# Lumina-Group/libzkp

Hardware: AMD Instinct MI355X
Metric: proofs/sec (whole node) + ms/proof p50, 4096-proof mixed batch (range / equality / membership / improvement) per MI355X (higher is better)
Workload: dtype u32/u64 integer limbs (10x25.5-bit GF(2^255-19), BN254 Fq on 9x29-bit limbs in the MSM loops and 10x26-bit elsewhere, 8x32-bit Fr and scalars mod l, 2x64-bit f128)

## Files before the change

__graft_entry__.py:

```python
import ctypes
import os
import re
import subprocess
import sys

ROOT = os.path.dirname(os.path.abspath(__file__))
CSRC = os.path.join(ROOT, "libzkp_amd", "csrc")
LIB = os.path.join(ROOT, "libzkp_amd", "lib", "libzkp_hip.so")
ORACLE_LIB = os.path.join(ROOT, "oracle", "_build", "libzkp_oracle.so")
EMUL_DIR = os.path.join(ROOT, "tests", "emul")


def _newer(target, sources):
    if not os.path.exists(target):
        return False
    t = os.path.getmtime(target)
    return all(os.path.getmtime(s) <= t for s in sources)


def _run(cmd, **kw):
    print("+", " ".join(cmd), flush=True)
    subprocess.check_call(cmd, **kw)


# ... 51 lines not shown
        _run(["g++", "-O2", "-std=c++17", "-fPIC", "-shared", "-o", so, src])


def build_emul_qap_lanes(force=False):
    out = os.path.join(EMUL_DIR, "_build")
    os.makedirs(out, exist_ok=True)
    exe, src = os.path.join(out, "emul_g16_qap_lanes"), os.path.join(EMUL_DIR, "emul_g16_qap_lanes.cpp")
    hdrs = [os.path.join(CSRC, f) for f in os.listdir(CSRC) if f.endswith(".h")]
    if force or not _newer(exe, hdrs + [src]):
        _run(["g++", "-O1", "-g", "-std=c++17", "-fsanitize=address,undefined", "-fno-sanitize-recover=undefined", "-o", exe, src])
    return exe


def build_emul_composites_seal_program(force=False):
    out = os.path.join(EMUL_DIR, "_build")
    os.makedirs(out, exist_ok=True)
    exe, src = os.path.join(out, "emul_composites_seal"), os.path.join(EMUL_DIR, "emul_composites_seal.cpp")
    hdrs = [os.path.join(CSRC, f) for f in os.listdir(CSRC) if f.endswith(".h")]
    if force or not _newer(exe, hdrs + [src]):
        _run(["g++", "-O1", "-g", "-std=c++17", "-fsanitize=address,undefined", "-fno-sanitize-recover=undefined", "-o", exe, src])
    return exe


def build_devtier(force=False):
    d = os.path.join(ROOT, "tests", "devtier")
    out = os.path.join(d, "_build")
    os.makedirs(out, exist_ok=True)
    hipcc = os.environ.get("HIPCC", "/opt/rocm/bin/hipcc")
    so = os.path.join(out, "libdevtier.so")
    if not os.path.exists(LIB):
        build_hip()
    if force or unit_is_stale(so, so + ".d", base=ROOT) or not _newer(so, [LIB]):
        _run([hipcc, "-O3", "-std=c++17", "--offload-arch=gfx950", "-fPIC", "-shared", "-MMD", "-MF", so + ".d", os.path.relpath(os.path.join(d, "devtier.hip"), ROOT), "-o", so,
              "-L" + os.path.dirname(LIB), "-lzkp_hip", "-Wl,-rpath,$ORIGIN/../../../libzkp_amd/lib"], cwd=ROOT)
    return so


def build_abi_caller(force=False):
    src = os.path.join(ROOT, "tests", "abi", "abi_call_all.cpp")
    out = os.path.join(ROOT, "tests", "abi", "_build")
    exe = os.path.join(out, "abi_call_all")
    os.makedirs(out, exist_ok=True)
    if force or not _newer(exe, [src, os.path.join(ROOT, "include", "libzkp_hip.h"), LIB]):
        _run(["g++", "-O1", "-std=c++17", "-pthread", "-D__HIP_PLATFORM_AMD__", "-I/opt/rocm/include", src, "-o", exe, "-L" + os.path.dirname(LIB), "-lzkp_hip",
              "-L/opt/rocm/lib", "-lamdhip64", "-Wl,-rpath,$ORIGIN/../../../libzkp_amd/lib", "-Wl,-rpath,/opt/rocm/lib"])
    return exe
# ... 21 lines not shown
        _run(["g++", "-O1", "-std=c++17", "-pthread", "-D__HIP_PLATFORM_AMD__", "-I/opt/rocm/include", src, "-o", exe, "-L" + os.path.dirname(LIB), "-lzkp_hip",
              "-L/opt/rocm/lib", "-lamdhip64", "-Wl,-rpath,$ORIGIN/../../../libzkp_amd/lib", "-Wl,-rpath,/opt/rocm/lib"])
    return exe


def build_abi_seal_caller(force=False):
    src = os.path.join(ROOT, "tests", "abi", "abi_call_seal.cpp")
    out = os.path.join(ROOT, "tests", "abi", "_build")
    exe = os.path.join(out, "abi_call_seal")
    os.makedirs(out, exist_ok=True)
    hdrs = [os.path.join(ROOT, "include", h) for h in ("libzkp_hip.h", "libzkp_hip_seal.h", "libzkp_hip_composites.h")]
    if force or not _newer(exe, [src, LIB] + hdrs):
        _run(["g++", "-O1", "-std=c++17", "-pthread", src, "-o", exe, "-L" + os.path.dirname(LIB), "-lzkp_hip",
              "-L/opt/rocm/lib", "-lamdhip64", "-Wl,-rpath,$ORIGIN/../../../libzkp_amd/lib", "-Wl,-rpath,/opt/rocm/lib"])
    return exe


def build():
    build_hip()
    build_oracle()
    build_emul()
    build_emul_qap_lanes()
    build_emul_composites_seal_program()
    build_devtier()
    build_abi_caller()
    build_abi_verify_caller()
    build_abi_statements_caller()
    build_abi_seal_caller()
    sys.path.insert(0, ROOT)
    import libzkp_amd
    from libzkp_amd import _native
    L = ctypes.CDLL(_native.LIB_PATH)
    for sym in _native.EXPORTS + _native.EXPORTS_VERIFY + _native.EXPORTS_BP_LOCALISE + _native.EXPORTS_COMPOSITES + _native.EXPORTS_STATEMENTS + _native.EXPORTS_SEAL:
        getattr(L, sym)
    print("build ok:", _native.LIB_PATH)


def smoke():
    import numpy as np
    sys.path.insert(0, ROOT)
    from libzkp_amd import _native
    L = _native.lib()
    _native.check(L.zkp_hip_init(0), "zkp_hip_init")
    orc = ctypes.CDLL(ORACLE_LIB)
    orc.zkp_oracle_init()
    n = 8
# ... 53 lines not shown
```

libzkp_amd/csrc/batch_impl.inc:

```
namespace {

struct PackView {
    uint32_t n;
    const uint64_t* src_off;
    const uint32_t* len_fixed;
    const uint32_t* dyn_ix;
    const uint8_t* dyn_kind;
    const int32_t* status_fixed;
    const uint32_t* dyn_len; const int32_t* dyn_status;
    uint32_t* len; int32_t* status; uint64_t* out_off;
    const uint8_t* arena; uint8_t* out;
};
__global__ void __launch_bounds__(256) k_batch_lens(PackView P) {
    const uint32_t i = blockIdx.x * 256 + threadIdx.x;
    if (i >= P.n) return;
    int32_t st = P.status_fixed[i];
    uint32_t l = P.len_fixed[i];
    if (st == 0 && l == LEN_DYN) {
        const uint32_t k = P.dyn_ix[i];
        l = P.dyn_len[k];
        if (P.dyn_kind[i] == DYN_LEN_STATUS) st = P.dyn_status[k];
        else if (l == 0) st = ZKP_HIP_PROOF_GENERATION_FAILED;
    }
    if (st != 0) l = 0;
// ... 199 lines not shown
    V.n = P.n; V.src_off = (const uint64_t*)(in + P.i_src); V.len_fixed = (const uint32_t*)(in + P.i_lenf); V.dyn_ix = (const uint32_t*)(in + P.i_dix);
    V.dyn_kind = in + P.i_dkind; V.status_fixed = (const int32_t*)(in + P.i_stf); V.dyn_len = (const uint32_t*)(ar + P.a_dlen); V.dyn_status = (const int32_t*)(ar + P.a_dst);
    V.len = (uint32_t*)(P.d_meta + P.m_len); V.status = (int32_t*)(P.d_meta + P.m_status); V.out_off = (uint64_t*)(P.d_meta + P.m_off);
    V.arena = ar; V.out = P.d_out;
    return V;
}

int launch_shard_enqueue(ShardPlan& P) {
    BatchState* BS = nullptr; int rc;
    if ((rc = batch_state(&BS))) return rc;
    const uint32_t n = P.n;
    uint32_t lane_ix = 0;
    if ((rc = pick_lane(*BS, &lane_ix))) return rc;
    BatchLane& LN = BS->lane[lane_ix];
    hipStream_t st = LN.main;
    uint8_t *in = P.d_in, *ar = P.d_arena;
    const VariantPlan &R = P.var[ZKP_HIP_OP_RANGE], &E = P.var[ZKP_HIP_OP_EQUALITY], &T = P.var[ZKP_HIP_OP_THRESHOLD], &M = P.var[ZKP_HIP_OP_MEMBERSHIP],
                      &I = P.var[ZKP_HIP_OP_IMPROVEMENT], &C = P.var[ZKP_HIP_OP_CONSISTENCY];
    trace_origin(st);
    if (P.arena_bytes) HIP_TRY(hipMemsetAsync(ar, 0, P.arena_bytes, st));
    if (T.rows) HIP_TRY(hipMemcpyAsync(ar + T.arena, P.thr_img.data(), P.thr_img.size(), hipMemcpyHostToDevice, st));
    if (C.rows) HIP_TRY(hipMemcpyAsync(ar + C.arena, P.con_img.data(), P.con_img.size(), hipMemcpyHostToDevice, st));
    HIP_TRY(hipEventRecord(LN.go, st));
    bool used[4] = {false, false, false, false};
    auto on_stream = [&](int k, auto body) -> int {
        hipStream_t s = nullptr; used[k] = true;
        int rcs;
        if ((rcs = lane_stream(*BS, k, &s))) return rcs;
        HIP_TRY(hipStreamWaitEvent(s, LN.go, 0));
        if ((rcs = body(s))) return rcs;
        HIP_TRY(hipEventRecord(LN.done[k], s));
        return 0;
    };
    if (R.rows || T.rows || C.rows) {
        static const int edg_prio = env_int("ZKP_HIP_EDG_PRIORITY", 1);
        struct PrioScope { int& r; PrioScope(int& ref, int v) : r(ref) { r = v; } ~PrioScope() { r = 0; } };
        PrioScope prio(dev().msm_prio_now, (E.rows + M.rows) && edg_prio ? 1 : 0);
        SubBatch& jobs_sb = dev().sub[0];
        if ((rc = on_stream(0, [&](hipStream_t s) -> int {
                int rcb;
                if (R.rows && (rcb = prove_range_device_locked(R.rows, (const uint64_t*)(in + P.i_rv), (const uint64_t*)(in + P.i_rmin), (const uint64_t*)(in + P.i_rmax), 6, in + P.i_rseed,
                                                               ar + R.arena, R.stride, (uint32_t*)(ar + P.a_dlen), (int32_t*)(ar + P.a_dst), s, nullptr, (int)lane_ix))) return rcb;
                if (T.rows && (rcb = run_jobs_on(jobs_sb, P.thrJ, in + P.i_tseed, ar + T.arena, 6, s))) return rcb;
                if (C.rows) {
                    if ((rcb = run_jobs_on(jobs_sb, P.conJ, in + P.i_cseed, ar + C.arena, 6, s))) return rcb;
                    k_consistency_digest<<<(C.rows + 63) / 64, 64, 0, s>>>(ar + C.arena, C.stride, (const uint32_t*)(in + P.i_ccount), (const uint32_t*)(in + P.i_clen), C.rows);
// ... 332 lines not shown
```

libzkp_amd/csrc/edg_kernels.hip:

```cpp
#include "edg_launch.h"
#include "msm_kernel.h"

struct EdGather {
    static constexpr uint32_t ACC_W = GE_W, DIG_PER_WORD = 2;
    static __device__ __forceinline__ int32_t digit(uint32_t word, uint32_t w) { return (int32_t)(int16_t)(word >> (16 * (w & 1u))); }
    using Acc = ge;
    static __device__ __forceinline__ Acc identity() { return ge_identity(); }
    static constexpr uint32_t GATHER_WAVES = 3; static constexpr int GATHER_PREFETCH = 2;
    static constexpr uint32_t GATHER_W = EDG_ENTRY_W, GATHER_STRIDE = EDG_SLOT_W, GATHER_PRIO = 0;
    using GAcc = ge;
    static __device__ __forceinline__ GAcc to_gather(const ge& a) { return a; }
    static __device__ __forceinline__ ge from_gather(const GAcc& a) { return a; }
    static __device__ __forceinline__ GAcc accumulate_entry(const GAcc& acc, int32_t d, const uint32_t* e) { return edg_accumulate(acc, d, e); }
    static __device__ __forceinline__ void store(uint32_t* p, uint32_t idx, uint32_t row, uint32_t rows, const Acc& a) { st_ge(p, idx, row, rows, a); }
    static __device__ __forceinline__ Acc load(const uint32_t* p, uint32_t idx, uint32_t row, uint32_t rows) { return ld_ge(p, idx, row, rows); }
    static __device__ __forceinline__ Acc add(const Acc& a, const Acc& b) { return ge_add(a, b); }
};
template __global__ void k_msm_gather<EdGather>(MsmView, uint32_t, uint32_t);
struct EdGatherPrio : EdGather { static constexpr uint32_t GATHER_PRIO = 1; };
template __global__ void k_msm_gather<EdGatherPrio>(MsmView, uint32_t, uint32_t);

uint32_t edg_msm_rows_per_block() { return 256; }
uint32_t edg_msm_blocks_per_cu() {
    int occ = 0;
    if (hipOccupancyMaxActiveBlocksPerMultiprocessor(&occ, k_msm_gather<EdGather>, 256, gather_lds_bytes<EdGather>()) != hipSuccess) { (void)hipGetLastError(); return 0; }
    return occ > 0 ? (uint32_t)occ : 0;
}
void edg_launch_msm(const MsmView& m, uint32_t ngroups, uint32_t nblocks, hipStream_t st, bool raised) {
    const uint32_t grid = ((nblocks + 7) / 8) * 8;
    if (raised) k_msm_gather<EdGatherPrio><<<grid, 256, gather_lds_bytes<EdGather>(), st>>>(m, ngroups, nblocks);
    else k_msm_gather<EdGather><<<grid, 256, gather_lds_bytes<EdGather>(), st>>>(m, ngroups, nblocks);
}

template <uint32_t WB> __global__ void __launch_bounds__(64) k_edg_bases(const uint32_t* gens, uint32_t* bases) {
    const uint32_t b = blockIdx.x * 64 + threadIdx.x;
    if (b < NBASE) edg_step_bases(edg_geom(WB), gens, bases, b);
}
template <uint32_t WB> __global__ void __launch_bounds__(64) k_edg_starts(const uint32_t* bases, uint32_t* starts) {
    constexpr EdgGeom g = edg_geom(WB);
    const uint32_t bw = blockIdx.x * 64 + threadIdx.x;
    if (bw < NBASE * g.nwin) edg_step_starts(g, bases, starts, bw);
}
template <uint32_t WB> __global__ void __launch_bounds__(256) k_edg_fill(const uint32_t* bases, const uint32_t* starts, uint32_t* table) {
    constexpr EdgGeom g = edg_geom(WB);
    const uint32_t t = blockIdx.x * 256 + threadIdx.x;
    if (t < NBASE * g.nwin * g.nseg) edg_step_fill(g, bases, starts, table, t / g.nseg, t % g.nseg);
}
template <uint32_t WB> __global__ void __launch_bounds__(256) k_edg_affine(uint32_t* table) {
    constexpr EdgGeom g = edg_geom(WB);
    const size_t grp = (size_t)blockIdx.x * 256 + threadIdx.x;
    if (grp < (size_t)NBASE * g.nwin * g.nent / EDG_INV) edg_step_affine(table, grp);
}
template <uint32_t WB> __global__ void __launch_bounds__(256) k_edg_check(const uint32_t* table, const uint32_t* gens, int* bad) {
    constexpr EdgGeom g = edg_geom(WB);
// ... 29 lines not shown
```

libzkp_amd/csrc/edg_launch.h:

```cpp
#pragma once
#include <hip/hip_runtime.h>
#include "edg.h"

uint32_t edg_msm_rows_per_block();
uint32_t edg_msm_blocks_per_cu();
void edg_launch_msm(const zkp::MsmView& m, uint32_t ngroups, uint32_t nblocks, hipStream_t st, bool raised = false);
void edg_launch_build(const zkp::EdgGeom& g, const uint32_t* d_gens, uint32_t* d_table, uint32_t* d_scratch, int* d_bad, hipStream_t st);
size_t edg_build_scratch_words(const zkp::EdgGeom& g);
void edg_launch_sum(const zkp::ReduceView& R, uint32_t* sums, hipStream_t st);
```

libzkp_amd/csrc/g16_impl.inc:

```

namespace {

struct G16Key {
    bool loaded = false;
    uint32_t n_inst = 0, n_wit = 0, nv = 0, n_rows = 0, m = 0, logm = 0;
    G16Circuit C{};
    std::vector<void*> allocs;
    uint32_t *table_g1 = nullptr, *table_g2 = nullptr;
    G16Radix rx = g16_radix(G16_WBITS_DEFAULT);
    int shared_tables = -1;
    uint64_t table_bytes = 0;
    struct Chunking { DevLayout lay; const uint32_t* corr = nullptr; const uint16_t* scal = nullptr; };
    std::vector<SlotList> targets_g1, targets_g2;
    std::vector<uint16_t> hscal_g1, hscal_g2;
    std::map<uint64_t, Chunking> lays_g1, lays_g2;
    uint64_t win_g1 = 0, win_g2 = 0;
    const uint32_t *init_g1 = nullptr, *init_g2 = nullptr;
    G16Vk vk{}; bool vk_ready = false;
    uint64_t vk_table_bytes = 0;
    bool verifier_only() const { return vk_ready && !loaded; }
    const uint32_t *vm_kconst = nullptr, *vm_lines = nullptr;
};
struct G16Run {
    void* buf = nullptr; size_t cap = 0; hipStream_t side = nullptr, side2 = nullptr; hipEvent_t ev[4] = {nullptr, nullptr, nullptr, nullptr};
// ... 355 lines not shown
    auto put = [](std::vector<uint8_t>& v, const uint8_t* p, size_t n) { v.insert(v.end(), p, p + n); };
    auto put_len = [](std::vector<uint8_t>& v, uint64_t n) { for (int i = 0; i < 8; i++) v.push_back((uint8_t)(n >> (8 * i))); };
    size_t o_abc = 3, o_a = o_abc + T.n_inst, o_b = o_a + nv, o_h = o_b + nv, o_l = o_h + (m - 1);
    vk.clear();
    put(vk, g1at(0), 64); put(vk, g2at(0), 128); put(vk, g2at(1), 128); put(vk, g2at(2), 128);
    put_len(vk, T.n_inst); put(vk, g1at(o_abc), 64ull * T.n_inst);
    pk = vk;
    put(pk, g1at(1), 64); put(pk, g1at(2), 64);
    put_len(pk, nv); put(pk, g1at(o_a), 64ull * nv);
    put_len(pk, nv); put(pk, g1at(o_b), 64ull * nv);
    put_len(pk, nv); put(pk, g2at(3), 128ull * nv);
    put_len(pk, m - 1); put(pk, g1at(o_h), 64ull * (m - 1));
    put_len(pk, T.n_wit); put(pk, g1at(o_l), 64ull * T.n_wit);
    return load_key_locked(kind, pk.data(), pk.size());
}

int launch_msm_key(bool g2, const G16Radix& rx, const G16Key::Chunking& ch, const uint32_t* table, const uint32_t* acc_init, uint32_t rows, const uint32_t* digits, uint32_t* partial, hipStream_t st) {
    const DevLayout& D = ch.lay;
    const MsmView m = g16_msm_view(rx, D, ch.scal, table, acc_init, rows, digits, partial);
    Device::KProf& K = dev().prof[g2 ? 2 : 1];
    hipEvent_t e1 = nullptr;
    int rc = prof_begin(K, st, &e1);
    if (rc) return rc;
    ZKP_TRACED(g2 ? "k_msm_gather<G2Msm>" : "k_msm_gather<G1Msm>", st, g16_launch_msm(g2, m, st));
    prof_end(K, st, e1, D.adds_per_row * rows);
    return 0;
}


int run_g16(int kind, uint32_t rows, const uint64_t* d_value, const uint64_t* d_set_vals, const uint32_t* d_set_len, const uint8_t* d_seeds,
            uint8_t* d_out, uint64_t stride, hipStream_t st, uint32_t lane = 0) {
    G16Key& K = g16s().key[kind];
    if (!K.loaded) return no_proving_key(K);
    const uint32_t nsc = g16_nscalars(K.nv, K.m);
    const G16Key::Chunking *c1 = nullptr, *c1c = nullptr, *c2 = nullptr;
    int rc;
    if ((rc = get_chunking(K, false, G16_PART_AB, rows, &c1)) || (rc = get_chunking(K, true, G16_PART_ALL, rows, &c2))) return rc;
    if ((rc = get_chunking(K, false, G16_PART_C, rows, &c1c))) return rc;
    size_t off = 0;
    auto sz = [&](size_t bytes) { size_t o = off; off += align_up(bytes); return o; };
    const size_t W = (size_t)32 * rows;
    const size_t o_z = sz(W * K.nv), o_sd = sz((size_t)K.rx.digw * 4 * rows * nsc), o_rs = sz(W * 2), o_p1 = sz((size_t)c1->lay.nchunks * G1_JAC_W * 4 * rows),
                 o_p1c = sz((size_t)c1c->lay.nchunks * G1_JAC_W * 4 * rows), o_p2 = sz((size_t)c2->lay.nchunks * G2_JAC_W * 4 * rows),
                 o_s1 = sz((size_t)3 * G1_JAC_W * 4 * rows), o_s2 = sz((size_t)G2_JAC_W * 4 * rows), o_t1 = sz((size_t)G16_CPARTS * G1_JAC_W * 4 * rows),
                 o_qe = sz((size_t)3 * 36 * K.m * rows);
    G16Run& RW = g16s().run[kind][lane & 1u];
    if (off > RW.cap) {
// ... 365 lines not shown
```

libzkp_amd/csrc/g16_kernels.hip:

```cpp
#include "g16_launch.h"
#include "msm_kernel.h"

struct G1Msm {
    static constexpr uint32_t ACC_W = G1_JAC_W, DIG_PER_WORD = 2;
    static __device__ __forceinline__ int32_t digit(uint32_t word, uint32_t w) { return (int32_t)(int16_t)(word >> (16 * (w & 1u))); }
    using Acc = g1_jac;
    static __device__ __forceinline__ Acc identity() { return jac_infinity<fq>(); }
    static constexpr uint32_t GATHER_WAVES = 3; static constexpr int GATHER_PREFETCH = 2;
    static constexpr uint32_t GATHER_W = 16, GATHER_STRIDE = 16, GATHER_PRIO = 0;
    using GAcc = g1_xyzz9;
    static __device__ __forceinline__ GAcc to_gather(const g1_jac& a) { return xyzz9_from_jac(a); }
    static __device__ __forceinline__ g1_jac from_gather(const GAcc& a) { return jac_from_xyzz9(a); }
    static __device__ __forceinline__ GAcc accumulate_entry(const GAcc& acc, int32_t d, const uint32_t* e) {
        g1_aff9 q{fq9_unpack8(e), fq9_unpack8(e + 8)};
        q.y = fq9_select(d < 0, fq9_neg_k<4>(q.y), q.y);
        return g1_mmadd9(acc, q);
    }
    static __device__ __forceinline__ void store(uint32_t* p, uint32_t idx, uint32_t row, uint32_t rows, const Acc& a) { st_g1_jac(p, idx, row, rows, a); }
    static __device__ __forceinline__ Acc load(const uint32_t* p, uint32_t idx, uint32_t row, uint32_t rows) { return ld_g1_jac(p, idx, row, rows); }
    static __device__ __forceinline__ Acc add(const Acc& a, const Acc& b) { return jac_add(a, b); }
};
struct G2Msm {
    static constexpr uint32_t ACC_W = G2_JAC_W, DIG_PER_WORD = 2;
    static __device__ __forceinline__ int32_t digit(uint32_t word, uint32_t w) { return (int32_t)(int16_t)(word >> (16 * (w & 1u))); }
// ... 133 lines not shown
#define QAP_PASS(D, N, H, T) if (dif == D && nst == N && head == H && tail == T) { k_g16_qap_pass<D, N, H, T><<<grid, QAP_TB, 0, st>>>(V, C, h, poly0); return; }
        G16_QAP_LANE_VARIANTS(QAP_PASS)
#undef QAP_PASS
        ok = false;
    });
    return ok ? hipSuccess : hipErrorInvalidValue;
}
void g16_launch_cparts(const G16View& V, const uint32_t* sum_g1, uint32_t* tmp_g1, hipStream_t st) {
    k_g16_cparts<<<dim3((V.rows + TW - 1) / TW, G16_CPARTS), TW, 0, st>>>(V, sum_g1, tmp_g1);
}
void g16_launch_final(const G16View& V, const uint32_t* sum_g1, const uint32_t* sum_g2, const uint32_t* tmp_g1, hipStream_t st) {
    k_g16_final<<<dim3((V.rows + TW - 1) / TW, 3), TW, 0, st>>>(V, sum_g1, sum_g2, tmp_g1);
}
void g16_launch_mimc(const uint64_t* values, uint32_t n, const uint32_t* mimc_c, uint8_t* out, hipStream_t st) { k_mimc_commit<<<(n + TW - 1) / TW, TW, 0, st>>>(values, n, mimc_c, out); }
void g16_launch_build_table(bool g2, const uint32_t* bases, uint32_t nslots, uint32_t* table, hipStream_t st, bool msm_form, const G16Radix& rx) {
    const uint32_t seg_len = rx.nent < G16_TABLE_SEG ? rx.nent : G16_TABLE_SEG;
    const uint32_t threads = nslots * (rx.slot_ent / seg_len);
    if (!g2) k_g16_build_table<fq, 20><<<(threads + TW - 1) / TW, TW, 0, st>>>(bases, nslots, table, msm_form ? 1u : 0u, rx);
    else k_g16_build_table<fq2, 40><<<(threads + TW - 1) / TW, TW, 0, st>>>(bases, nslots, table, msm_form ? 1u : 0u, rx);
}
uint32_t g16_table_entry_words(bool g2, bool msm_form) { return msm_form ? (g2 ? G2Msm::GATHER_W : G1Msm::GATHER_W) : (g2 ? 40u : 20u); }
uint32_t g16_msm_rows_per_block(bool) { return 256u; }
uint32_t g16_msm_blocks_per_cu(bool g2) { return g2 ? G2Msm::GATHER_WAVES : G1Msm::GATHER_WAVES; }
void g16_launch_msm(bool g2, const MsmView& m, hipStream_t st) {
    const uint32_t ngroups = (m.rows + 255u) / 256u, nblocks = m.nchunks * ngroups, grid = ((nblocks + 7) / 8) * 8;
    if constexpr (gather_lds_bytes<G2Msm>() > 0 || gather_lds_bytes<G1Msm>() > 0) {
        if (gather_lds_bytes<G1Msm>()) (void)hipFuncSetAttribute(reinterpret_cast<const void*>(k_msm_gather<G1Msm>), hipFuncAttributeMaxDynamicSharedMemorySize, (int)gather_lds_bytes<G1Msm>());
        if (gather_lds_bytes<G2Msm>()) (void)hipFuncSetAttribute(reinterpret_cast<const void*>(k_msm_gather<G2Msm>), hipFuncAttributeMaxDynamicSharedMemorySize, (int)gather_lds_bytes<G2Msm>());
    }
    if (!g2) k_msm_gather<G1Msm><<<grid, 256, gather_lds_bytes<G1Msm>(), st>>>(m, ngroups, nblocks);
    else k_msm_gather<G2Msm><<<grid, 256, gather_lds_bytes<G2Msm>(), st>>>(m, ngroups, nblocks);
}
void g16_launch_sum(bool g2, const ReduceView& R, uint32_t* sums, hipStream_t st) {
    const dim3 grid((R.rows + G16_SUM_ROWS - 1) / G16_SUM_ROWS, R.ntargets);
    if (!g2) k_sum_t<G1Msm, G16_SUM_ROWS, G16_SUM_TB><<<grid, G16_SUM_TB, 0, st>>>(R, sums);
    else k_sum_t<G2Msm, G16_SUM_ROWS, G16_SUM_TB><<<grid, G16_SUM_TB, 0, st>>>(R, sums);
}
void g16_launch_serialize(bool g2, const uint32_t* jac, uint32_t rows, uint8_t* out, hipStream_t st) { k_g16_serialize<<<(rows + TW - 1) / TW, TW, 0, st>>>(g2, jac, rows, out); }
```

libzkp_amd/csrc/g16_launch.h:

```cpp
#pragma once
#include <hip/hip_runtime.h>
#include "g16_steps.h"
#include "bp_steps.h"

void g16_launch_witness(const zkp::G16View& V, hipStream_t st);
void g16_launch_zdigits(const zkp::G16View& V, hipStream_t st);
hipError_t g16_launch_qap(const zkp::G16View& V, const zkp::G16Circuit& C, hipStream_t st);
void g16_launch_cparts(const zkp::G16View& V, const uint32_t* sum_g1, uint32_t* tmp_g1, hipStream_t st);
void g16_launch_final(const zkp::G16View& V, const uint32_t* sum_g1, const uint32_t* sum_g2, const uint32_t* tmp_g1, hipStream_t st);
void g16_launch_mimc(const uint64_t* values, uint32_t n, const uint32_t* mimc_c, uint8_t* out, hipStream_t st);
void g16_launch_build_table(bool g2, const uint32_t* bases, uint32_t nslots, uint32_t* table, hipStream_t st, bool msm_form, const zkp::G16Radix& rx);
uint32_t g16_table_entry_words(bool g2, bool msm_form);
uint32_t g16_msm_rows_per_block(bool g2);
uint32_t g16_msm_blocks_per_cu(bool g2);
void g16_launch_msm(bool g2, const zkp::MsmView& m, hipStream_t st);
void g16_launch_sum(bool g2, const zkp::ReduceView& R, uint32_t* sums, hipStream_t st);
void g16_launch_serialize(bool g2, const uint32_t* jac, uint32_t rows, uint8_t* out, hipStream_t st);
```

libzkp_amd/csrc/msm_kernel.h:

```cpp
#pragma once
#include <hip/hip_runtime.h>
#include "bp_steps.h"

using namespace zkp;
static constexpr int TW = 64;
static constexpr int TB = 256;


template <class T> constexpr size_t gather_lds_bytes() { return T::GATHER_PREFETCH < 0 ? (size_t)4 * 2 * (T::GATHER_W / 4) * 64 * 16 : 0; }
template <class T>
__global__ void __launch_bounds__(256, T::GATHER_WAVES) k_msm_gather(MsmView m, uint32_t ngroups, uint32_t nblocks) {
    constexpr uint32_t V4 = T::GATHER_W / 4;
    constexpr uint32_t SV4 = T::GATHER_STRIDE / 4;
    const uint32_t tid = threadIdx.x;
    const uint32_t per_xcd = (nblocks + 7) / 8;
    const uint32_t linear = (blockIdx.x & 7u) * per_xcd + (blockIdx.x >> 3);
    if (linear >= nblocks) return;
    const uint32_t chunk = linear / ngroups, group = linear % ngroups;
    const uint32_t row = group * 256u + tid;
    const bool active = row < m.rows;
    const uint32_t st0 = m.chunk_step0[chunk], left = m.chunk_step0[chunk + 1] - st0;
    const uint2* const steps = reinterpret_cast<const uint2*>(m.steps) + st0;
    typename T::GAcc acc = T::to_gather(m.acc_init ? T::load(m.acc_init, 0, 0, 1) : T::identity());
    const uint4* const table4 = reinterpret_cast<const uint4*>(m.table);
    auto digit_word = [&](const uint2 ds) -> uint32_t { return active ? m.digits[(size_t)(ds.y >> 1) * m.rows + row] : 0u; };
    auto entry_of = [&](const uint2 ds, int32_t d) -> const uint4* { return table4 + ((uint64_t)ds.x + (uint32_t)((d < 0 ? -d : d) - 1)) * SV4; };
    if (left == 0) { if (active) T::store(m.partial, chunk, row, m.rows, T::from_gather(acc)); return; }
    if constexpr (T::GATHER_PREFETCH < 0) {
#if defined(__HIP_DEVICE_COMPILE__)
        extern __shared__ uint4 gather_lds[];
        const uint32_t wave = tid >> 6, lane = tid & 63u;
        uint4* const wbuf = gather_lds + (size_t)wave * (2u * V4 * 64u);
// ... 81 lines not shown
```

libzkp_amd/csrc/zkp_hip.hip:

```cpp
#include <hip/hip_runtime.h>
#include <mutex>
#include <memory>
#include <algorithm>
#include <map>
#include <array>
#include <type_traits>
#include <atomic>
#include <thread>
#include <condition_variable>
#include <functional>
#include <deque>
#include <new>
#include <exception>
#include <cstring>
#include <string>
#include <vector>
#include <cstdio>
#include <cstdlib>
#include <cmath>
#include <chrono>
#include <sys/random.h>
#include "bp_layout.h"
#include "g16_steps.h"
#include "sha256_host.h"
#include "g16_circuit.h"
#include "g16_keyblob.h"
#include "g16_share.h"
#include "msm_kernel.h"
#include "g16_launch.h"
#include "g16_verify_launch.h"
#include "stark_launch.h"
#include "bpv_launch.h"
#include "edg_launch.h"
#include "batch_self_check.h"
#include "batch_plan.h"
#include "verify_shards.h"
#include "venv_steps.h"
#include "composite_steps.h"
#include "composite_seal.h"
#include "vst_steps.h"
#include "../../include/libzkp_hip_verify.h"
#include "../../include/libzkp_hip_bp_localise.h"
#include "../../include/libzkp_hip_composites.h"
#include "../../include/libzkp_hip_seal.h"


__global__ void __launch_bounds__(TB) k_build_range(JobBuf J, uint32_t n, const uint64_t* value, const uint64_t* mn, const uint64_t* mx, uint32_t lg,
                                                    uint8_t* out, uint64_t stride, uint32_t* out_len, int32_t* status) {
    ZKP_RAISE_PRIO();
    const uint32_t op = blockIdx.x * TB + threadIdx.x;
    if (op < n) step_build_range(J, op, value, mn, mx, lg, out, stride, out_len, status);
}
__global__ void __launch_bounds__(TB) k_ctask(CtView T) {
    ZKP_RAISE_PRIO();
    const uint32_t c = blockIdx.x * TB + threadIdx.x;
    if (c < T.C) step_ctask(T, c);
}
__global__ void __launch_bounds__(TB) k_tape(BpView V) {
// ... 193 lines not shown
constexpr int MAXT = 8;
struct LayoutSet { std::vector<DevLayout> cand; uint32_t max_chunks = 0; };

struct SubBatch {
    hipStream_t stream = nullptr;
    hipEvent_t start = nullptr, done = nullptr;
    hipStream_t side = nullptr;
    hipEvent_t side_go = nullptr, side_done = nullptr;
    bool used = false;
    bool borrowed = false;
    void* ws = nullptr;
    uint32_t capM = 0, capC = 0, cap_chunks = 0;
};
constexpr uint32_t NSLOTS = 2;

struct G16State; struct StarkState; struct VfyState; struct BatchState;
struct Device {
    int index = 0, hip_dev = 0;
    std::mutex mu;
    bool ready = false;
    uint64_t generation = 0;
    int num_cu = 256;
    int msm_prio_now = 0;
    hipStream_t stream = nullptr;
    uint32_t* d_edg_table = nullptr;
    EdgGeom edg = {0, 0, 0, 0, 0};
    bool bp_ready = false;
    int edg_blocks_per_cu = 3;
    struct Family { LayoutSet p1, rd[6]; bool ready = false; };
    Family fam[4];
    LayoutSet p2, ct;
    uint32_t max_chunks = 0;
    SubBatch sub[NSLOTS];
    uint32_t next_slot = 0;
    DevPool pool;
    G16State* g16 = nullptr; StarkState* stark = nullptr; VfyState* vfy = nullptr; BatchState* batch = nullptr;
    bool profiling = false;
    struct KProf {
        std::vector<std::pair<hipEvent_t, hipEvent_t>> ev_pool; size_t ev_used = 0;
        double ms = 0; uint64_t launches = 0, adds = 0;
    };
    KProf prof[3];
    struct HostCounter { double ms = 0; uint64_t a = 0, b = 0; };
    HostCounter host[ZKP_HIP_COUNTER_VERIFY_MIXED - ZKP_HIP_COUNTER_G16_VERIFY + 1];
    HostCounter& counter(int which) { return host[which - ZKP_HIP_COUNTER_G16_VERIFY]; }
    struct BpLocaliseCounter { double ms = 0; uint64_t failed_checks = 0, segment_checks = 0, jobs_again = 0; } bp_localise;
// ... 47 lines not shown
int env_int(const char* name, int dflt) { const char* v = getenv(name); return v && *v ? atoi(v) : dflt; }
int stream_priority(int level) {
    int least = 0, greatest = 0; (void)hipDeviceGetStreamPriorityRange(&least, &greatest);
    return level == 0 ? greatest : level == 2 ? least : (least + greatest) / 2;
}
int bp_priority_level() { static const int v = env_int("ZKP_HIP_BP_PRIORITY", 1); return v; }
int stark_priority_level() { static const int v = env_int("ZKP_HIP_STARK_PRIORITY", 1); return v; }
int g16_priority_level() { static const int v = env_int("ZKP_HIP_G16_PRIORITY", 2); return v; }

int prof_begin(Device::KProf& K, hipStream_t st, hipEvent_t* e1) {
    *e1 = nullptr;
    if (!dev().profiling) return 0;
    if (K.ev_used == K.ev_pool.size()) { hipEvent_t a, b; HIP_TRY(hipEventCreate(&a)); HIP_TRY(hipEventCreate(&b)); K.ev_pool.push_back({a, b}); }
    HIP_TRY(hipEventRecord(K.ev_pool[K.ev_used].first, st));
    *e1 = K.ev_pool[K.ev_used].second; K.ev_used++;
    return 0;
}
void prof_end(Device::KProf& K, hipStream_t st, hipEvent_t e1, uint64_t adds) {
    if (!e1) return;
    (void)hipEventRecord(e1, st); K.launches++; K.adds += adds;
}

struct Trace {
    struct Rec { const char* name; hipStream_t st; hipEvent_t a, b; };
    std::vector<Rec> recs;
    std::vector<hipEvent_t> pool; size_t used = 0;
    hipEvent_t origin = nullptr; bool have_origin = false;
    std::string path;
    hipEvent_t take() { if (used == pool.size()) { hipEvent_t e = nullptr; (void)hipEventCreate(&e); pool.push_back(e); } return pool[used++]; }
};
Trace* trace_state() {
    Device& D = dev();
    if (D.trace) return D.trace->path.empty() ? nullptr : D.trace;
    D.trace = new Trace();
    const char* v = getenv("ZKP_HIP_TRACE");
    if (v && *v) D.trace->path = v;
    return D.trace->path.empty() ? nullptr : D.trace;
}
void trace_origin(hipStream_t st) {
    Trace* T = trace_state(); if (!T) return;
    if (!T->origin) (void)hipEventCreate(&T->origin);
    (void)hipEventRecord(T->origin, st); T->have_origin = true;
}
struct TraceMark {
    Trace* T; Trace::Rec r;
    TraceMark(const char* name, hipStream_t st) : T(trace_state()) { if (T) { r = {name, st, T->take(), T->take()}; (void)hipEventRecord(r.a, st); } }
    ~TraceMark() { if (T) { (void)hipEventRecord(r.b, r.st); T->recs.push_back(r); } }
};
#define ZKP_TRACED(name, st, ...) do { TraceMark tm_(name, st); __VA_ARGS__; } while (0)
void trace_dump() {
    Trace* T = trace_state(); if (!T || T->recs.empty()) return;
    (void)hipDeviceSynchronize();
    FILE* f = fopen(T->path.c_str(), "a");
    if (f) {
        std::map<hipStream_t, int> ids;
        fputs("[", f);
        bool first = true;
        for (auto& r : T->recs) {
            float ta = 0, tb = 0;
            if (!T->have_origin || hipEventElapsedTime(&ta, T->origin, r.a) != hipSuccess || hipEventElapsedTime(&tb, T->origin, r.b) != hipSuccess) continue;
            const int id = ids.emplace(r.st, (int)ids.size()).first->second;
            fprintf(f, "%s[\"%s\", %d, %.4f, %.4f]", first ? "" : ", ", r.name, id, ta, tb); first = false;
        }
        fputs("]\n", f);
        fclose(f);
    }
    (void)hipGetLastError();
    T->recs.clear(); T->used = 0; T->have_origin = false;
}
void trace_release() {
    Trace* T = dev().trace; if (!T) return;
    for (auto e : T->pool) (void)hipEventDestroy(e);
    if (T->origin) (void)hipEventDestroy(T->origin);
    delete T; dev().trace = nullptr;
}

int upload_layout(DevLayout& D, const MsmLayout& L, const GatherShape* shape = nullptr, const uint16_t* slot_scalar = nullptr) {
    D.nslots = L.nslots(); D.nchunks = L.nchunks(); D.ntargets = L.ntargets();
    D.adds_per_row = 0; for (uint8_t x : L.slot_nwin) D.adds_per_row += x;
    D.max_chunk_windows = 0;
    for (uint32_t c = 0; c < D.nchunks; c++) if (L.chunk_nwin[c] > D.max_chunk_windows) D.max_chunk_windows = L.chunk_nwin[c];
    D.max_target_chunks = 0;
    for (uint32_t t = 0; t < D.ntargets; t++) {
        const uint32_t k = L.target_chunk_begin[t + 1] - L.target_chunk_begin[t];
        if (k > D.max_target_chunks) D.max_target_chunks = k;
// ... 389 lines not shown
}

int ensure_workspace(SubBatch& sb, uint32_t M, uint32_t C) {
    if (M <= sb.capM && C <= sb.capC && dev().max_chunks <= sb.cap_chunks && sb.ws) return 0;
    if (sb.ws) { HIP_TRY(hipDeviceSynchronize()); HIP_TRY(hipFree(sb.ws)); sb.ws = nullptr; }
    const uint32_t nm = M > sb.capM ? M : sb.capM, nc = C > sb.capC ? C : sb.capC;
    const size_t bytes = carve(nullptr, nm, nc, dev().max_chunks, nullptr);
    HIP_TRY(hipMalloc(&sb.ws, bytes));
    sb.capM = nm; sb.capC = nc; sb.cap_chunks = dev().max_chunks;
    return 0;
}

int launch_msm(const DevLayout& D, uint32_t rows, const uint32_t* digits, uint32_t* partial, hipStream_t st) {
    MsmView m; m.rows = rows; m.nslots = D.nslots; m.nchunks = D.nchunks; m.table = dev().d_edg_table; m.digits = digits;
    m.slot_base = D.slot_base; m.slot_scalar = nullptr; m.slot_nwin = D.slot_nwin; m.chunk_begin = D.chunk_begin; m.chunk_win0 = D.chunk_win0; m.chunk_nwin = D.chunk_nwin; m.partial = partial; m.acc_init = nullptr;
    hipEvent_t e1 = nullptr;
    int rc = prof_begin(dev().prof[0], st, &e1);
    if (rc) return rc;
    {
        const EdgGeom& g = dev().edg;
        m.nwin = g.nwin; m.nent = g.nent; m.digw = DIGW; m.slot_ent = g.nwin * g.nent; m.uneven = 0;
        m.steps = D.steps; m.chunk_step0 = D.chunk_step0;
        const uint32_t tb = edg_msm_rows_per_block(), ngroups = (rows + tb - 1) / tb, nblocks = D.nchunks * ngroups;
        ZKP_TRACED("k_msm_gather<EdGather>", st, edg_launch_msm(m, ngroups, nblocks, st, dev().msm_prio_now != 0));
    }
    prof_end(dev().prof[0], st, e1, D.adds_per_row * rows);
    return 0;
}
void launch_sum_ed(const ReduceView& R, uint32_t* sums, hipStream_t st) {
    k_sum_t<EdMsm, ED_SUM_ROWS, ED_SUM_TB><<<dim3((R.rows + ED_SUM_ROWS - 1) / ED_SUM_ROWS, R.ntargets), ED_SUM_TB, 0, st>>>(R, sums);
}
int launch_reduce(const DevLayout& D, uint32_t rows, const uint32_t* partial, uint32_t* sums, uint32_t* enc, const uint64_t* out_off, uint8_t* out, hipStream_t st) {
    ReduceView R; R.rows = rows; R.ntargets = D.ntargets; R.partial = partial; R.target_chunk_begin = D.target_chunk_begin;
    R.enc = enc; R.out_off = out_off; R.out = out; R.corr = nullptr;
    ZKP_TRACED("k_sum_t<EdMsm>", st, launch_sum_ed(R, sums, st));
    ZKP_TRACED("k_encode", st, k_encode<<<dim3((rows + TW - 1) / TW, D.ntargets), TW, 0, st>>>(R, sums));
    return 0;
}
int msm_and_encode(const LayoutSet& S, uint32_t rows, const uint32_t* digits, uint32_t* partial, uint32_t* sums, uint32_t* enc, const uint64_t* out_off, uint8_t* out, hipStream_t st) {
    const DevLayout& D = pick_layout(S, rows);
    int rc = launch_msm(D, rows, digits, partial, st);
    if (rc) return rc;
    return launch_reduce(D, rows, partial, sums, enc, out_off, out, st);
}

int run_pipeline(const Ws& w, uint32_t M, uint32_t C, hipStream_t st, SubBatch& lane) {
    int rc;
// ... 367 lines not shown
```

Measured before the change: 355,400.

## Reserve extra LDS on G1 gather MSM to cap its per-CU occupancy in mixed batches

Adds an occupancy planner that, for mixed batches (range plus equality/membership), pads the dynamic LDS of the G1 Groth16 gather MSM kernel so at most two blocks fit per CU. This leaves CU resources for concurrently running kernels on other streams (EdDSA gather, QAP, sums). The gather launch helpers now take the reserve and set the max dynamic shared memory attribute only when it is needed. The risk is that the G1 MSM loses throughput from lower occupancy if co-scheduling does not make up for it.

```diff
diff --git a/__graft_entry__.py b/__graft_entry__.py
--- a/__graft_entry__.py
+++ b/__graft_entry__.py
@@ -97,6 +97,15 @@
     return exe
 
 
+def build_emul_occupancy_plan(force=False):
+    out = os.path.join(EMUL_DIR, "_build")
+    os.makedirs(out, exist_ok=True)
+    exe, src = os.path.join(out, "emul_occupancy_plan"), os.path.join(EMUL_DIR, "emul_occupancy_plan.cpp")
+    if force or not _newer(exe, [os.path.join(CSRC, "occupancy_plan.h"), src]):
+        _run(["g++", "-O1", "-g", "-std=c++17", "-fsanitize=address,undefined", "-fno-sanitize-recover=undefined", "-o", exe, src])
+    return exe
+
+
 def build_devtier(force=False):
     d = os.path.join(ROOT, "tests", "devtier")
     out = os.path.join(d, "_build")
@@ -164,6 +173,7 @@
     build_emul()
     build_emul_qap_lanes()
     build_emul_composites_seal_program()
+    build_emul_occupancy_plan()
     build_devtier()
     build_abi_caller()
     build_abi_verify_caller()
diff --git a/libzkp_amd/csrc/batch_impl.inc b/libzkp_amd/csrc/batch_impl.inc
--- a/libzkp_amd/csrc/batch_impl.inc
+++ b/libzkp_amd/csrc/batch_impl.inc
@@ -245,6 +245,9 @@
     if (T.rows) HIP_TRY(hipMemcpyAsync(ar + T.arena, P.thr_img.data(), P.thr_img.size(), hipMemcpyHostToDevice, st));
     if (C.rows) HIP_TRY(hipMemcpyAsync(ar + C.arena, P.con_img.data(), P.con_img.size(), hipMemcpyHostToDevice, st));
     HIP_TRY(hipEventRecord(LN.go, st));
+    static const bool occ_on = env_int("ZKP_HIP_OCCUPANCY_PLAN", 1) != 0;
+    struct OccScope { OccPlan& r; OccScope(OccPlan& ref, const OccPlan& p) : r(ref) { r = p; } ~OccScope() { r = OccPlan{}; } };
+    OccScope occ(dev().occ_now, occ_plan(OccBatch{R.rows + T.rows + C.rows, E.rows, M.rows, I.rows}, occ_on));
     bool used[4] = {false, false, false, false};
     auto on_stream = [&](int k, auto body) -> int {
         hipStream_t s = nullptr; used[k] = true;
diff --git a/libzkp_amd/csrc/edg_kernels.hip b/libzkp_amd/csrc/edg_kernels.hip
--- a/libzkp_amd/csrc/edg_kernels.hip
+++ b/libzkp_amd/csrc/edg_kernels.hip
@@ -26,10 +26,10 @@
     if (hipOccupancyMaxActiveBlocksPerMultiprocessor(&occ, k_msm_gather<EdGather>, 256, gather_lds_bytes<EdGather>()) != hipSuccess) { (void)hipGetLastError(); return 0; }
     return occ > 0 ? (uint32_t)occ : 0;
 }
-void edg_launch_msm(const MsmView& m, uint32_t ngroups, uint32_t nblocks, hipStream_t st, bool raised) {
+void edg_launch_msm(const MsmView& m, uint32_t ngroups, uint32_t nblocks, hipStream_t st, bool raised, uint32_t reserve) {
     const uint32_t grid = ((nblocks + 7) / 8) * 8;
-    if (raised) k_msm_gather<EdGatherPrio><<<grid, 256, gather_lds_bytes<EdGather>(), st>>>(m, ngroups, nblocks);
-    else k_msm_gather<EdGather><<<grid, 256, gather_lds_bytes<EdGather>(), st>>>(m, ngroups, nblocks);
+    if (raised) k_msm_gather<EdGatherPrio><<<grid, 256, gather_launch_lds<EdGatherPrio>(k_msm_gather<EdGatherPrio>, reserve), st>>>(m, ngroups, nblocks);
+    else k_msm_gather<EdGather><<<grid, 256, gather_launch_lds<EdGather>(k_msm_gather<EdGather>, reserve), st>>>(m, ngroups, nblocks);
 }
 
 template <uint32_t WB> __global__ void __launch_bounds__(64) k_edg_bases(const uint32_t* gens, uint32_t* bases) {
diff --git a/libzkp_amd/csrc/edg_launch.h b/libzkp_amd/csrc/edg_launch.h
--- a/libzkp_amd/csrc/edg_launch.h
+++ b/libzkp_amd/csrc/edg_launch.h
@@ -4,7 +4,7 @@
 
 uint32_t edg_msm_rows_per_block();
 uint32_t edg_msm_blocks_per_cu();
-void edg_launch_msm(const zkp::MsmView& m, uint32_t ngroups, uint32_t nblocks, hipStream_t st, bool raised = false);
+void edg_launch_msm(const zkp::MsmView& m, uint32_t ngroups, uint32_t nblocks, hipStream_t st, bool raised = false, uint32_t reserve = 0);
 void edg_launch_build(const zkp::EdgGeom& g, const uint32_t* d_gens, uint32_t* d_table, uint32_t* d_scratch, int* d_bad, hipStream_t st);
 size_t edg_build_scratch_words(const zkp::EdgGeom& g);
 void edg_launch_sum(const zkp::ReduceView& R, uint32_t* sums, hipStream_t st);
diff --git a/libzkp_amd/csrc/g16_impl.inc b/libzkp_amd/csrc/g16_impl.inc
--- a/libzkp_amd/csrc/g16_impl.inc
+++ b/libzkp_amd/csrc/g16_impl.inc
@@ -401,7 +401,8 @@
     hipEvent_t e1 = nullptr;
     int rc = prof_begin(K, st, &e1);
     if (rc) return rc;
-    ZKP_TRACED(g2 ? "k_msm_gather<G2Msm>" : "k_msm_gather<G1Msm>", st, g16_launch_msm(g2, m, st));
+    const uint32_t reserve = dev().occ_now.reserve[g2 ? OCC_G2 : OCC_G1];
+    ZKP_TRACED_GATHER(g2 ? "k_msm_gather<G2Msm>" : "k_msm_gather<G1Msm>", st, reserve, g16_launch_msm(g2, m, st, reserve));
     prof_end(K, st, e1, D.adds_per_row * rows);
     return 0;
 }
diff --git a/libzkp_amd/csrc/g16_kernels.hip b/libzkp_amd/csrc/g16_kernels.hip
--- a/libzkp_amd/csrc/g16_kernels.hip
+++ b/libzkp_amd/csrc/g16_kernels.hip
@@ -179,14 +179,10 @@
 uint32_t g16_table_entry_words(bool g2, bool msm_form) { return msm_form ? (g2 ? G2Msm::GATHER_W : G1Msm::GATHER_W) : (g2 ? 40u : 20u); }
 uint32_t g16_msm_rows_per_block(bool) { return 256u; }
 uint32_t g16_msm_blocks_per_cu(bool g2) { return g2 ? G2Msm::GATHER_WAVES : G1Msm::GATHER_WAVES; }
-void g16_launch_msm(bool g2, const MsmView& m, hipStream_t st) {
+void g16_launch_msm(bool g2, const MsmView& m, hipStream_t st, uint32_t reserve) {
     const uint32_t ngroups = (m.rows + 255u) / 256u, nblocks = m.nchunks * ngroups, grid = ((nblocks + 7) / 8) * 8;
-    if constexpr (gather_lds_bytes<G2Msm>() > 0 || gather_lds_bytes<G1Msm>() > 0) {
-        if (gather_lds_bytes<G1Msm>()) (void)hipFuncSetAttribute(reinterpret_cast<const void*>(k_msm_gather<G1Msm>), hipFuncAttributeMaxDynamicSharedMemorySize, (int)gather_lds_bytes<G1Msm>());
-        if (gather_lds_bytes<G2Msm>()) (void)hipFuncSetAttribute(reinterpret_cast<const void*>(k_msm_gather<G2Msm>), hipFuncAttributeMaxDynamicSharedMemorySize, (int)gather_lds_bytes<G2Msm>());
-    }
-    if (!g2) k_msm_gather<G1Msm><<<grid, 256, gather_lds_bytes<G1Msm>(), st>>>(m, ngroups, nblocks);
-    else k_msm_gather<G2Msm><<<grid, 256, gather_lds_bytes<G2Msm>(), st>>>(m, ngroups, nblocks);
+    if (!g2) k_msm_gather<G1Msm><<<grid, 256, gather_launch_lds<G1Msm>(k_msm_gather<G1Msm>, reserve), st>>>(m, ngroups, nblocks);
+    else k_msm_gather<G2Msm><<<grid, 256, gather_launch_lds<G2Msm>(k_msm_gather<G2Msm>, reserve), st>>>(m, ngroups, nblocks);
 }
 void g16_launch_sum(bool g2, const ReduceView& R, uint32_t* sums, hipStream_t st) {
     const dim3 grid((R.rows + G16_SUM_ROWS - 1) / G16_SUM_ROWS, R.ntargets);
diff --git a/libzkp_amd/csrc/g16_launch.h b/libzkp_amd/csrc/g16_launch.h
--- a/libzkp_amd/csrc/g16_launch.h
+++ b/libzkp_amd/csrc/g16_launch.h
@@ -13,6 +13,6 @@
 uint32_t g16_table_entry_words(bool g2, bool msm_form);
 uint32_t g16_msm_rows_per_block(bool g2);
 uint32_t g16_msm_blocks_per_cu(bool g2);
-void g16_launch_msm(bool g2, const zkp::MsmView& m, hipStream_t st);
+void g16_launch_msm(bool g2, const zkp::MsmView& m, hipStream_t st, uint32_t reserve = 0);
 void g16_launch_sum(bool g2, const zkp::ReduceView& R, uint32_t* sums, hipStream_t st);
 void g16_launch_serialize(bool g2, const uint32_t* jac, uint32_t rows, uint8_t* out, hipStream_t st);
diff --git a/libzkp_amd/csrc/msm_kernel.h b/libzkp_amd/csrc/msm_kernel.h
--- a/libzkp_amd/csrc/msm_kernel.h
+++ b/libzkp_amd/csrc/msm_kernel.h
@@ -8,6 +8,11 @@
 
 
 template <class T> constexpr size_t gather_lds_bytes() { return T::GATHER_PREFETCH < 0 ? (size_t)4 * 2 * (T::GATHER_W / 4) * 64 * 16 : 0; }
+template <class T> size_t gather_launch_lds(void (*kernel)(MsmView, uint32_t, uint32_t), uint32_t reserve) {
+    const size_t bytes = gather_lds_bytes<T>() + reserve;
+    if (bytes >= 64 * 1024) (void)hipFuncSetAttribute(reinterpret_cast<const void*>(kernel), hipFuncAttributeMaxDynamicSharedMemorySize, (int)bytes);
+    return bytes;
+}
 template <class T>
 __global__ void __launch_bounds__(256, T::GATHER_WAVES) k_msm_gather(MsmView m, uint32_t ngroups, uint32_t nblocks) {
     constexpr uint32_t V4 = T::GATHER_W / 4;
diff --git a/libzkp_amd/csrc/occupancy_plan.h b/libzkp_amd/csrc/occupancy_plan.h
--- /dev/null
+++ b/libzkp_amd/csrc/occupancy_plan.h
@@ -0,0 +1,64 @@
+#pragma once
+#include <cstdint>
+
+namespace zkp {
+
+constexpr uint32_t OCC_VGPRS_PER_SIMD = 512, OCC_VGPR_GRANULE = 8, OCC_LDS_PER_CU = 160u * 1024u, OCC_LDS_GRANULE = 1024;
+
+enum OccKernelId : uint32_t { OCC_G1 = 0, OCC_G2 = 1, OCC_ED = 2, OCC_NGATHER = 3, OCC_QAP = 3, OCC_QAP_WIDE = 4, OCC_SUM_G1 = 5, OCC_SUM_G2 = 6, OCC_SUM_ED = 7, OCC_STARK = 8, OCC_NKERNELS = 9 };
+struct OccKernel { uint32_t vgprs, lds_bytes, waves; };
+constexpr OccKernel OCC_KERNELS[OCC_NKERNELS] = {
+    {134, 0, 4},
+    {243, 65536, 4},
+    {156, 0, 4},
+    {80, 0, 4},
+    {90, 0, 4},
+    {189, 15360, 4},
+    {401, 30720, 4},
+    {209, 20480, 4},
+    {101, 21808, 1},
+};
+
+struct OccBatch { uint32_t range_rows, equality_rows, membership_rows, stark_rows; };
+struct OccCaps { uint32_t cap[OCC_NGATHER]; };
+struct OccSet { uint32_t count[OCC_NKERNELS]; };
+struct OccPlan { uint32_t cap[OCC_NGATHER], reserve[OCC_NGATHER]; };
+
+constexpr uint32_t occ_vgpr_alloc(uint32_t vgprs) { return (vgprs + OCC_VGPR_GRANULE - 1) / OCC_VGPR_GRANULE * OCC_VGPR_GRANULE; }
+
+constexpr uint32_t occ_reserve_bytes(uint32_t cap, uint32_t lds_bytes) {
+    if (cap == 0) return 0;
+    const uint32_t need = OCC_LDS_PER_CU / (cap + 1) + 1;
+    const uint32_t size = (need + OCC_LDS_GRANULE - 1) / OCC_LDS_GRANULE * OCC_LDS_GRANULE;
+    return size > lds_bytes ? size - lds_bytes : 0;
+}
+
+inline uint32_t occ_set_vgprs(const OccSet& s) {
+    uint32_t v = 0;
+    for (uint32_t i = 0; i < OCC_NKERNELS; i++) v += s.count[i] * occ_vgpr_alloc(OCC_KERNELS[i].vgprs) * ((OCC_KERNELS[i].waves + 3) / 4);
+    return v;
+}
+inline uint32_t occ_set_lds(const OccPlan& p, const OccSet& s) {
+    uint32_t b = 0;
+    for (uint32_t i = 0; i < OCC_NKERNELS; i++) b += s.count[i] * (OCC_KERNELS[i].lds_bytes + (i < OCC_NGATHER ? p.reserve[i] : 0));
+    return b;
+}
+inline bool occ_set_fits(const OccPlan& p, const OccSet& s) { return occ_set_vgprs(s) <= OCC_VGPRS_PER_SIMD && occ_set_lds(p, s) <= OCC_LDS_PER_CU; }
+
+inline OccPlan occ_plan_for_caps(const OccCaps& c) {
+    OccPlan p{};
+    for (uint32_t i = 0; i < OCC_NGATHER; i++) { p.cap[i] = c.cap[i]; p.reserve[i] = occ_reserve_bytes(c.cap[i], OCC_KERNELS[i].lds_bytes); }
+    return p;
+}
+
+constexpr OccCaps OCC_MIXED_CAPS = {{2, 0, 0}};
+constexpr uint32_t OCC_MIXED_NSETS = 4;
+constexpr OccSet OCC_MIXED_SETS[OCC_MIXED_NSETS] = {{{2, 0, 1, 1, 0, 0, 0, 0, 0}}, {{2, 0, 0, 0, 2, 0, 0, 0, 0}}, {{2, 0, 0, 0, 0, 1, 0, 0, 0}}, {{1, 1, 0, 0, 1, 0, 0, 0, 0}}};
+
+inline bool occ_batch_is_mixed(const OccBatch& b) { return b.range_rows != 0 && (b.equality_rows != 0 || b.membership_rows != 0); }
+inline OccPlan occ_plan(const OccBatch& b, bool enabled) {
+    if (!enabled || !occ_batch_is_mixed(b)) return OccPlan{};
+    return occ_plan_for_caps(OCC_MIXED_CAPS);
+}
+
+}
diff --git a/libzkp_amd/csrc/zkp_hip.hip b/libzkp_amd/csrc/zkp_hip.hip
--- a/libzkp_amd/csrc/zkp_hip.hip
+++ b/libzkp_amd/csrc/zkp_hip.hip
@@ -34,6 +34,7 @@
 #include "edg_launch.h"
 #include "batch_self_check.h"
 #include "batch_plan.h"
+#include "occupancy_plan.h"
 #include "verify_shards.h"
 #include "venv_steps.h"
 #include "composite_steps.h"
@@ -273,6 +274,7 @@
     uint64_t generation = 0;
     int num_cu = 256;
     int msm_prio_now = 0;
+    OccPlan occ_now{};
     hipStream_t stream = nullptr;
     uint32_t* d_edg_table = nullptr;
     EdgGeom edg = {0, 0, 0, 0, 0};
@@ -366,7 +368,7 @@
 }
 
 struct Trace {
-    struct Rec { const char* name; hipStream_t st; hipEvent_t a, b; };
+    struct Rec { const char* name; hipStream_t st; hipEvent_t a, b; int64_t reserve; };
     std::vector<Rec> recs;
     std::vector<hipEvent_t> pool; size_t used = 0;
     hipEvent_t origin = nullptr; bool have_origin = false;
@@ -388,10 +390,11 @@
 }
 struct TraceMark {
     Trace* T; Trace::Rec r;
-    TraceMark(const char* name, hipStream_t st) : T(trace_state()) { if (T) { r = {name, st, T->take(), T->take()}; (void)hipEventRecord(r.a, st); } }
+    TraceMark(const char* name, hipStream_t st, int64_t reserve = -1) : T(trace_state()) { if (T) { r = {name, st, T->take(), T->take(), reserve}; (void)hipEventRecord(r.a, st); } }
     ~TraceMark() { if (T) { (void)hipEventRecord(r.b, r.st); T->recs.push_back(r); } }
 };
 #define ZKP_TRACED(name, st, ...) do { TraceMark tm_(name, st); __VA_ARGS__; } while (0)
+#define ZKP_TRACED_GATHER(name, st, reserve_bytes, ...) do { TraceMark tm_(name, st, (int64_t)(reserve_bytes)); __VA_ARGS__; } while (0)
 void trace_dump() {
     Trace* T = trace_state(); if (!T || T->recs.empty()) return;
     (void)hipDeviceSynchronize();
@@ -404,7 +407,9 @@
             float ta = 0, tb = 0;
             if (!T->have_origin || hipEventElapsedTime(&ta, T->origin, r.a) != hipSuccess || hipEventElapsedTime(&tb, T->origin, r.b) != hipSuccess) continue;
             const int id = ids.emplace(r.st, (int)ids.size()).first->second;
-            fprintf(f, "%s[\"%s\", %d, %.4f, %.4f]", first ? "" : ", ", r.name, id, ta, tb); first = false;
+            fprintf(f, "%s[\"%s\", %d, %.4f, %.4f", first ? "" : ", ", r.name, id, ta, tb); first = false;
+            if (r.reserve >= 0) fprintf(f, ", %lld", (long long)r.reserve);
+            fputs("]", f);
         }
         fputs("]\n", f);
         fclose(f);
@@ -840,7 +845,7 @@
         m.nwin = g.nwin; m.nent = g.nent; m.digw = DIGW; m.slot_ent = g.nwin * g.nent; m.uneven = 0;
         m.steps = D.steps; m.chunk_step0 = D.chunk_step0;
         const uint32_t tb = edg_msm_rows_per_block(), ngroups = (rows + tb - 1) / tb, nblocks = D.nchunks * ngroups;
-        ZKP_TRACED("k_msm_gather<EdGather>", st, edg_launch_msm(m, ngroups, nblocks, st, dev().msm_prio_now != 0));
+        ZKP_TRACED_GATHER("k_msm_gather<EdGather>", st, dev().occ_now.reserve[OCC_ED], edg_launch_msm(m, ngroups, nblocks, st, dev().msm_prio_now != 0, dev().occ_now.reserve[OCC_ED]));
     }
     prof_end(dev().prof[0], st, e1, D.adds_per_row * rows);
     return 0;
```

Result: no change. 358,100, median of 3 (+0.8%).
